# Xiaoming-Zhao/PointNav-VO

Hardware: AMD Instinct MI355X
Metric: RGB-D frame-pair VO inferences/s @341x192 (higher is better)
Workload: dtype f32

## Files before the change

pointnav-vo_amd/csrc/conv_x3.hip:

```cpp
#include <cmath>
#include <cstdio>
#include <cstdlib>
#include <cstring>

#include "pnvo_internal.h"

namespace pnvo {

typedef float f32x16 __attribute__((ext_vector_type(16)));
typedef float f32x4 __attribute__((ext_vector_type(4)));
typedef float f32x2 __attribute__((ext_vector_type(2)));
typedef __bf16 bf16x8 __attribute__((ext_vector_type(8)));
typedef __bf16 bf16x2 __attribute__((ext_vector_type(2)));
typedef _Float16 f16x8 __attribute__((ext_vector_type(8)));
typedef _Float16 f16x2 __attribute__((ext_vector_type(2)));
typedef unsigned u32x4 __attribute__((ext_vector_type(4)));

namespace {
__device__ __forceinline__ unsigned pack2(float a, float b) {
  const bf16x2 r = __builtin_convertvector(f32x2{a, b}, bf16x2);
  return __builtin_bit_cast(unsigned, r);
}
__device__ __forceinline__ unsigned pack2h(float a, float b) {
  const f16x2 r = __builtin_convertvector(f32x2{a, b}, f16x2);
  return __builtin_bit_cast(unsigned, r);
}
__device__ __forceinline__ float lo_f(unsigned u) { return __builtin_bit_cast(float, u << 16); }
__device__ __forceinline__ float hi_f(unsigned u) { return __builtin_bit_cast(float, u & 0xffff0000u); }
}

constexpr int x3_wpe(int mw, int nw, int np, bool dsf = false) {
  return dsf ? (mw * nw >= 6 ? 1 : (mw * nw >= 2 ? 2 : 3)) : ((np == 2 && mw * nw <= 2) ? 3 : 2);
}

template <int KS, int STRIDE, int MODE, int MW, int NW, int NP, bool DSF = false, bool W8 = false, bool KSW = false, bool M16 = false>
__global__ __launch_bounds__(W8 ? 512 : 256) __attribute__((amdgpu_waves_per_eu(W8 ? 2 : x3_wpe(MW, NW, NP, DSF), W8 ? 2 : x3_wpe(MW, NW, NP, DSF)))) void conv_x3_kernel(const ConvX3Args p) {
  constexpr int NTH = W8 ? 512 : 256, NWV = NTH / 64;
  constexpr int EMW = KSW ? 1 : MW;
  constexpr int NWT = M16 ? NW / 2 : NW;
  constexpr int TW = M16 ? (MW * NW + 3) / 4 : MW * NW;
  static_assert(!M16 || (NP == 2 && KS == 3 && STRIDE == 1 && !DSF && !KSW && NW % 2 == 0), "16x16x32 flavour: float16-piece 3x3 stride-1 convs, whole N-tiles");
  static_assert(!KSW || (NW == 1 && NP == 2 && KS == 3 && !DSF && !W8), "K split over the waves: float16-piece 3x3 convs, one N-tile");
  static_assert(!DSF || (KS == 3 && STRIDE == 2 && NP == 2 && (MODE == 0 || MODE == 2)), "the downsample rides on a float16-piece 3x3 stride-2 conv");
  extern __shared__ __attribute__((aligned(16))) unsigned char lds[];
  constexpr int PSTEP = KS == 1 ? STRIDE : 1;
  constexpr int CS = KS == 1 ? 1 : STRIDE;
  constexpr int PAD = KS / 2;
  const int lane = threadIdx.x & 63;
  const int wave = __builtin_amdgcn_readfirstlane(threadIdx.x >> 6);

  const int ntiles = p.B * p.tiles_r * p.tiles_c;
  const int chunk = (ntiles + 7) >> 3;
  int bid = (int)(blockIdx.x & 7) * chunk + (int)(blockIdx.x >> 3);
  if (bid >= ntiles) return;
  const int tci = bid % p.tiles_c;
  bid /= p.tiles_c;
  const int tri = bid % p.tiles_r;
  const int n = bid / p.tiles_r;
  const int r0 = tri * p.TR, c0 = tci * p.TC;
  const int hi0 = r0 * STRIDE - PAD, wi0 = c0 * STRIDE - PAD;
  const int mdl = (p.grp_end0 > 0 && n >= p.grp_end0) + (p.grp_end1 > 0 && n >= p.grp_end1);
  const unsigned short *g_wpk = mdl == 0 ? p.wpk : p.wpk_g[mdl - 1];
  const unsigned short *g_ds_wpk = mdl == 0 ? p.ds_wpk : p.ds_wpk_g[mdl - 1];
  const float g_oscale = mdl == 0 ? p.oscale : p.oscale_g[mdl - 1], g_ds_oscale = mdl == 0 ? p.ds_oscale : p.ds_oscale_g[mdl - 1];
  const float *g_gamma = mdl == 0 ? p.gn_gamma : p.gn_gamma_g[mdl - 1], *g_beta = mdl == 0 ? p.gn_beta : p.gn_beta_g[mdl - 1];
  const float *g_ds_gamma = mdl == 0 ? p.ds_gamma : p.ds_gamma_g[mdl - 1], *g_ds_beta = mdl == 0 ? p.ds_beta : p.ds_beta_g[mdl - 1];
  const int PR = p.PR, PC = p.PC, CK = p.CK;
  const int pitch = CK * 2 + 16;
  const int plane = PR * PC * pitch;
  const int npix = p.TR * p.TC;
  const int tab_off = KSW ? max(NP * plane, 4 * MW * 4096) : NP * plane;
  unsigned *qtab = reinterpret_cast<unsigned *>(lds + tab_off);
  unsigned *otab = qtab + p.MT * 32;
  for (int e = (int)threadIdx.x; e < p.MT * 32; e += NTH) {
    const int q = min(e, npix - 1);
    const int tr = q / p.TC, tc = q - tr * p.TC;
    qtab[e] = (unsigned)(((tr * CS) * PC + tc * CS) * pitch);
    const bool ok = e < npix && r0 + tr < p.Ho && c0 + tc < p.Wo;
    otab[e] = (unsigned)((tr * p.Wo + tc) * p.COUTP) | (ok ? 0u : 0x80000000u);
  }

  const int wn = p.wn;
  const int wave_m = wave / wn;
  const int wave_n = (wave & (wn - 1)) + (int)blockIdx.y * wn;
  const int ntt = p.COUTP >> 5, kct = p.CIN >> 4;

  f32x16 acc[MW][NW];
#pragma unroll
  for (int i = 0; i < MW; ++i)
#pragma unroll
    for (int j = 0; j < NW; ++j)
#pragma unroll
      for (int r = 0; r < 16; ++r) acc[i][j][r] = 0.f;
  f32x4 acc16[M16 ? MW : 1][M16 ? NW : 1];
  const int mt16 = (npix + 15) >> 4;
  const int m16_row = (mt16 + NWV / wn - 1) / (NWV / wn), m16_sub0 = wave_m * m16_row;
  const bool m16_last = m16_sub0 + MW <= mt16 && MW <= m16_row;
  if (M16) {
#pragma unroll
    for (int i = 0; i < MW; ++i)
#pragma unroll
      for (int j = 0; j < NW; ++j) acc16[M16 ? i : 0][M16 ? j : 0] = f32x4{0.f, 0.f, 0.f, 0.f};
  }
  f32x16 accd[DSF ? MW : 1][DSF ? NW : 1];
  if (DSF) {
#pragma unroll
    for (int i = 0; i < MW; ++i)
#pragma unroll
      for (int j = 0; j < NW; ++j)
#pragma unroll
        for (int r = 0; r < 16; ++r) accd[DSF ? i : 0][DSF ? j : 0][r] = 0.f;
  }

  float in_mul = 1.f, in_div = 1.f;
  const bool in_scaled = NP == 2 && p.in_absmax != nullptr;
  if (in_scaled) {
    unsigned mb = p.in_absmax[(threadIdx.x & 63) * 16];
#pragma unroll
    for (int d = 32; d >= 1; d >>= 1) mb = max(mb, (unsigned)__shfl_xor((int)mb, d));
    const int e = mb != 0u ? (int)((mb >> 23) & 0xffu) - 126 : 14;
    in_mul = __builtin_bit_cast(float, (unsigned)(14 - e + 127) << 23);
    in_div = __builtin_bit_cast(float, (unsigned)(e - 14 + 127) << 23);
  }
  const int G = CK >> 3;
  const int cg = threadIdx.x & (G - 1), pl = threadIdx.x / G, PS = NTH / G;
  const int dr = PS / PC, dc = PS - dr * PC;
  const int nppix = PR * PC;

  unsigned long long c_stage = 0, c_mm = 0, t_0 = __builtin_readcyclecounter(), r_0 = wall_clock64();
  for (int ck0 = 0; ck0 < p.CIN; ck0 += CK) {
    unsigned long long t_a = __builtin_readcyclecounter();
    if (ck0 > 0) __syncthreads();
    {
      f32x4 sc0, sc1, sh0, sh1, rs0, rs1, rt0, rt1;
      const bool res_ss = MODE == 2 && p.res_scale != nullptr;
      auto load_ss = [&]() {
        if (MODE >= 1) {
          const float *ps = p.in_scale + (long)n * p.CIN + ck0 + 8 * cg;
          const float *pt = p.in_shift + (long)n * p.CIN + ck0 + 8 * cg;
          sc0 = *reinterpret_cast<const f32x4 *>(ps);
          sc1 = *reinterpret_cast<const f32x4 *>(ps + 4);
          sh0 = *reinterpret_cast<const f32x4 *>(pt);
          sh1 = *reinterpret_cast<const f32x4 *>(pt + 4);
        }
        if (res_ss) {
          const float *ps = p.res_scale + (long)n * p.CIN + ck0 + 8 * cg;
          const float *pt = p.res_shift + (long)n * p.CIN + ck0 + 8 * cg;
          rs0 = *reinterpret_cast<const f32x4 *>(ps);
          rs1 = *reinterpret_cast<const f32x4 *>(ps + 4);
          rt0 = *reinterpret_cast<const f32x4 *>(pt);
          rt1 = *reinterpret_cast<const f32x4 *>(pt + 4);
        }
      };
      load_ss();
      int pr = pl / PC, pc = pl - pr * PC;
      const long img = ((long)n * p.H * p.W) * p.CIN + ck0 + 8 * cg;
      const float *xb = p.x + img;
      struct Round {
        f32x4 v[2][2], w[2][2];
        unsigned off[2];
        int gofs[2];
        bool ok[2], in[2], own[2];
      };
      auto fetch = [&](int pix, Round &r) {
#pragma unroll
        for (int k = 0; k < 2; ++k) {
          const int hi = hi0 + pr * PSTEP, wi = wi0 + pc * PSTEP;
          r.ok[k] = pix + k * PS < nppix;
          r.in[k] = r.ok[k] && hi >= 0 && hi < p.H && wi >= 0 && wi < p.W;
          r.off[k] = (unsigned)((pr * PC + pc) * pitch + 16 * cg);
          r.v[k][0] = r.v[k][1] = f32x4{0.f, 0.f, 0.f, 0.f};
          if (MODE >= 2) {
            r.own[k] = r.in[k] && p.xout != nullptr && blockIdx.y == 0 && pr >= PAD && pr < PAD + p.TR * CS && pc >= PAD && pc < PAD + p.TC * CS;
            r.gofs[k] = (hi * p.W + wi) * p.CIN;
          }
          if (r.in[k]) {
            const float *src = xb + ((long)hi * p.W + wi) * p.CIN;
            r.v[k][0] = *reinterpret_cast<const f32x4 *>(src);
            r.v[k][1] = *reinterpret_cast<const f32x4 *>(src + 4);
            if (MODE == 2) {
              const float *rsrc = p.res + img + ((long)hi * p.W + wi) * p.CIN;
              r.w[k][0] = *reinterpret_cast<const f32x4 *>(rsrc);
              r.w[k][1] = *reinterpret_cast<const f32x4 *>(rsrc + 4);
            }
          }
          pr += dr;
          pc += dc;
          if (pc >= PC) {
            pc -= PC;
            pr += 1;
          }
        }
      };
      auto split_store = [&](const Round &r) {
#pragma unroll
        for (int k = 0; k < 2; ++k) {
          if (!r.ok[k]) continue;
          float f[8];
#pragma unroll
          for (int e = 0; e < 8; ++e) {
            float t = r.v[k][e >> 2][e & 3];
            if (MODE == 1) {
              const f32x4 &sc = e < 4 ? sc0 : sc1, &sh = e < 4 ? sh0 : sh1;
              t = r.in[k] ? fmaxf(__builtin_fmaf(t, sc[e & 3], sh[e & 3]), 0.f) : 0.f;
            }
            if (MODE == 3) {
              const f32x4 &sc = e < 4 ? sc0 : sc1, &sh = e < 4 ? sh0 : sh1;
              int key = __builtin_bit_cast(int, t);
              key = key >= 0 ? key : key ^ 0x7fffffff;
              t = r.in[k] ? fmaxf(__builtin_fmaf(__builtin_bit_cast(float, key), __builtin_fabsf(sc[e & 3]), sh[e & 3]), 0.f) : 0.f;
            }
            if (MODE == 2) {
              const f32x4 &sc = e < 4 ? sc0 : sc1, &sh = e < 4 ? sh0 : sh1;
              float u = r.w[k][e >> 2][e & 3];
              if (res_ss) u = __builtin_fmaf(u, (e < 4 ? rs0 : rs1)[e & 3], (e < 4 ? rt0 : rt1)[e & 3]);
              t = r.in[k] ? fmaxf(__builtin_fmaf(t, sc[e & 3], sh[e & 3]) + u, 0.f) : 0.f;
            }
            f[e] = t;
          }
          if (MODE >= 2 && r.own[k]) {
            float *dst = p.xout + img + r.gofs[k];
            *reinterpret_cast<f32x4 *>(dst) = f32x4{f[0], f[1], f[2], f[3]};
            *reinterpret_cast<f32x4 *>(dst + 4) = f32x4{f[4], f[5], f[6], f[7]};
          }
          if (NP == 2) {
            if (in_scaled) {
#pragma unroll
              for (int e = 0; e < 8; ++e) f[e] *= in_mul;
            }
            u32x4 o0, o1;
#pragma unroll
            for (int e = 0; e < 4; ++e) {
              const float a = f[2 * e], b = f[2 * e + 1];
              const f16x2 h = __builtin_convertvector(f32x2{a, b}, f16x2);
              o0[e] = __builtin_bit_cast(unsigned, h);
              o1[e] = pack2h(a - (float)h[0], b - (float)h[1]);
            }
            *reinterpret_cast<u32x4 *>(lds + r.off[k]) = o0;
            *reinterpret_cast<u32x4 *>(lds + plane + r.off[k]) = o1;
            continue;
          }
          u32x4 o0, o1, o2;
#pragma unroll
          for (int e = 0; e < 4; ++e) {
            const float a = f[2 * e], b = f[2 * e + 1];
            const unsigned h = pack2(a, b);
            const float ra = a - lo_f(h), rb = b - hi_f(h);
            const unsigned m = pack2(ra, rb);
            o0[e] = h;
            o1[e] = m;
            o2[e] = pack2(ra - lo_f(m), rb - hi_f(m));
          }
          *reinterpret_cast<u32x4 *>(lds + r.off[k]) = o0;
          *reinterpret_cast<u32x4 *>(lds + plane + r.off[k]) = o1;
          *reinterpret_cast<u32x4 *>(lds + 2 * plane + r.off[k]) = o2;
        }
      };
      constexpr bool PIPE = !((MODE == 2 && (TW >= 6 || (M16 && !W8) || x3_wpe(MW, NW, NP) == 3 || DSF)) || (DSF && MW * NW == 4));
      if (TW <= 2 && !(MODE == 2 && (x3_wpe(MW, NW, NP) == 3 || DSF))) {
        for (int pix = pl; pix < nppix; pix += 6 * PS) {
          Round r0, r1, r2;
          fetch(pix, r0);
          fetch(pix + 2 * PS, r1);
          fetch(pix + 4 * PS, r2);
          split_store(r0);
          split_store(r1);
          split_store(r2);
        }
      } else if (PIPE) {
        Round cur, nxt;
        fetch(pl, cur);
        for (int pix = pl; pix < nppix; pix += 2 * PS) {
          const bool more = pix + 2 * PS < nppix;
          if (more) fetch(pix + 2 * PS, nxt);
          split_store(cur);
          if (more) cur = nxt;
        }
      } else {
        for (int pix = pl; pix < nppix; pix += 2 * PS) {
          Round cur;
          fetch(pix, cur);
          split_store(cur);
        }
      }
    }
    __syncthreads();
    unsigned long long t_b = __builtin_readcyclecounter();
    c_stage += t_b - t_a;

    if constexpr (M16) {
      unsigned aoff[MW];
#pragma unroll
      for (int i = 0; i < MW; ++i) {
        const int sub = min(m16_sub0 + i, mt16 - 1);
        aoff[i] = qtab[sub * 16 + (lane & 15)] + (unsigned)((lane >> 4) * 16);
      }
      const int kcc = CK >> 4, kcp = CK >> 5;
      const int nsteps = KS * KS * kcp;
      const unsigned kstep = (unsigned)ntt * (NP * 1024u);
      const char *wb_n = reinterpret_cast<const char *>(g_wpk) + (long)(ck0 >> 4) * kstep;
      unsigned toff_n = 0;
      int kc_n = 0, kw_n = 0;
      auto advance = [&]() {
        ++kc_n;
        toff_n += 64;
        wb_n += 2 * kstep;
        if (kc_n == kcp) {
          kc_n = 0;
          toff_n += (unsigned)(pitch - kcp * 64);
          wb_n += (long)(kct - kcc) * kstep;
          if (++kw_n == KS) {
            kw_n = 0;
            toff_n += (unsigned)((PC - KS) * pitch);
          }
        }
      };
      const int kg = lane >> 4;
      unsigned voff[NW];
#pragma unroll
      for (int j = 0; j < NW; ++j)
        voff[j] = (unsigned)min(wave_n * NWT + (j >> 1), ntt - 1) * (NP * 1024u) + (unsigned)(kg >> 1) * kstep +
                  (unsigned)((kg & 1) * 32 + 16 * (j & 1) + (lane & 15)) * 16u;
      auto loadA = [&](int i, u32x4 (*a)[MW]) {
#pragma unroll
        for (int pc = 0; pc < NP; ++pc) a[pc][i] = *reinterpret_cast<const u32x4 *>(lds + pc * plane + aoff[i] + toff_n);
      };
      auto loadB = [&](u32x4 (*b)[NW]) {
#pragma unroll
        for (int j = 0; j < NW; ++j)
#pragma unroll
          for (int pc = 0; pc < NP; ++pc) b[pc][j] = *reinterpret_cast<const u32x4 *>(wb_n + (size_t)voff[j] + pc * 1024);
      };
      auto step = [&](u32x4 (*a)[MW], const u32x4 (*b)[NW]) {
#pragma unroll
        for (int i = 0; i < MW; ++i) {
          if (i == MW - 1 && !m16_last) break;
          constexpr int TA[3] = {1, 0, 0}, TB[3] = {0, 1, 0};
#pragma unroll
          for (int jt = 0; jt < NWT; ++jt)
#pragma unroll
            for (int t = 0; t < 3; ++t)
#pragma unroll
              for (int j = 2 * jt; j < 2 * jt + 2; ++j)
                acc16[M16 ? i : 0][M16 ? j : 0] = __builtin_amdgcn_mfma_f32_16x16x32_f16(__builtin_bit_cast(f16x8, a[TA[t]][i]), __builtin_bit_cast(f16x8, b[TB[t]][M16 ? j : 0]),
                                                                                         acc16[M16 ? i : 0][M16 ? j : 0], 0, 0, 0);
          __builtin_amdgcn_sched_barrier(0);
          loadA(i, a);
          __builtin_amdgcn_sched_barrier(0);
        }
      };
      u32x4 a[NP][MW], b0[NP][NW], b1[NP][NW];
      loadB(b0);
#pragma unroll
      for (int i = 0; i < MW; ++i) loadA(i, a);
      advance();
#pragma unroll 1
      for (int s = 0; s < nsteps; s += 2) {
        loadB(b1);
        __builtin_amdgcn_sched_barrier(0);
        step(a, b0);
        if (s + 2 < nsteps) advance();
        if (s + 1 < nsteps) {
          loadB(b0);
          __builtin_amdgcn_sched_barrier(0);
          step(a, b1);
          if (s + 3 < nsteps) advance();
        }
      }
    } else {
    unsigned aoff[MW];
#pragma unroll
    for (int i = 0; i < MW; ++i) {
      const int mt = min(KSW ? i : wave_m * MW + i, p.MT - 1);
      aoff[i] = qtab[mt * 32 + (lane & 31)] + (unsigned)((lane >> 5) * 16);
    }
    const int kcc = CK >> 4;
    const int nsteps = KS * KS * kcc;
    const unsigned kstep = (unsigned)ntt * (NP * 1024u);
    const char *wb_n = reinterpret_cast<const char *>(g_wpk) + (long)(ck0 >> 4) * kstep;
    unsigned toff_n = 0;
    int kc_n = 0, kw_n = 0;
    auto advance = [&]() {
      ++kc_n;
      toff_n += 32;
      wb_n += kstep;
      if (kc_n == kcc) {
        kc_n = 0;
        toff_n += (unsigned)(pitch - kcc * 32);
        wb_n += (long)(kct - kcc) * kstep;
        if (++kw_n == KS) {
          kw_n = 0;
          toff_n += (unsigned)((PC - KS) * pitch);
        }
      }
    };
    constexpr bool RING = NP == 2 && KS == 3 && MW * NW <= 2;
    const char *wb_b = wb_n;
    int kc_b = 0;
    auto advanceB = [&]() {
      wb_b += kstep;
      if (++kc_b == kcc) {
        kc_b = 0;
        wb_b += (long)(kct - kcc) * kstep;
      }
    };
    unsigned voff[NW];
#pragma unroll
    for (int j = 0; j < NW; ++j) voff[j] = (unsigned)min(wave_n * NW + j, ntt - 1) * (NP * 1024u) + (unsigned)lane * 16u;
    auto loadBr = [&](u32x4 (*b)[NW]) {
#pragma unroll
      for (int j = 0; j < NW; ++j)
#pragma unroll
        for (int pc = 0; pc < NP; ++pc) b[pc][j] = *reinterpret_cast<const u32x4 *>(wb_b + (size_t)voff[j] + pc * 1024);
    };
    auto loadA = [&](int i, u32x4 (*a)[MW]) {
#pragma unroll
      for (int pc = 0; pc < NP; ++pc) a[pc][i] = *reinterpret_cast<const u32x4 *>(lds + pc * plane + aoff[i] + toff_n);
    };
    auto loadB = [&](u32x4 (*b)[NW]) {
#pragma unroll
      for (int j = 0; j < NW; ++j)
#pragma unroll
        for (int pc = 0; pc < NP; ++pc) b[pc][j] = *reinterpret_cast<const u32x4 *>(wb_n + (size_t)voff[j] + pc * 1024);
    };
    auto step = [&](u32x4 (*a)[MW], const u32x4 (*b)[NW]) {
#pragma unroll
      for (int i = 0; i < MW; ++i) {
#pragma unroll
        for (int j = 0; j < NW; ++j) {
          if (NP == 2) {
            constexpr int TA[3] = {1, 0, 0}, TB[3] = {0, 1, 0};
#pragma unroll
            for (int t = 0; t < 3; ++t)
              acc[i][j] = __builtin_amdgcn_mfma_f32_32x32x16_f16(__builtin_bit_cast(f16x8, a[TA[t]][i]),
                                                                 __builtin_bit_cast(f16x8, b[TB[t]][j]), acc[i][j], 0, 0, 0);
          } else {
            constexpr int TA[6] = {1, 2, 0, 1, 0, 0}, TB[6] = {1, 0, 2, 0, 1, 0};
#pragma unroll
            for (int t = 0; t < 6; ++t)
              acc[i][j] = __builtin_amdgcn_mfma_f32_32x32x16_bf16(__builtin_bit_cast(bf16x8, a[TA[t]][i]),
                                                                  __builtin_bit_cast(bf16x8, b[TB[t]][j]), acc[i][j], 0, 0, 0);
          }
        }
        __builtin_amdgcn_sched_barrier(0);
        loadA(i, a);
        __builtin_amdgcn_sched_barrier(0);
      }
    };
    u32x4 a[NP][MW], b0[NP][NW], b1[NP][NW];
    u32x4 bd0[DSF ? NP : 1][NW], bd1[DSF ? NP : 1][NW];
    auto loadBd = [&](u32x4 (*b)[NW], int kc) {
      const char *wd = reinterpret_cast<const char *>(g_ds_wpk) + (long)((ck0 >> 4) + kc) * kstep;
#pragma unroll
      for (int j = 0; j < NW; ++j)
#pragma unroll
        for (int pc = 0; pc < NP; ++pc) b[pc][j] = *reinterpret_cast<const u32x4 *>(wd + (size_t)voff[j] + pc * 1024);
    };
    if constexpr (KSW) {
      const int s0 = (wave * nsteps) >> 2, s1 = ((wave + 1) * nsteps) >> 2;
      {
        const int tap = s0 / kcc, kc = s0 - tap * kcc, kh = tap / KS, kw = tap - kh * KS;
        kc_n = kc;
        kw_n = kw;
        toff_n = (unsigned)((kh * PC + kw) * pitch + kc * 32);
        wb_n += ((long)tap * kct + kc) * kstep;
        kc_b = kc;
        wb_b = wb_n;
      }
      u32x4 br[3][NP][NW];
      int fb = s0;
      auto fetchB = [&](u32x4 (*bq)[NW]) {
        loadBr(bq);
        if (++fb < s1) advanceB();
      };
      fetchB(br[0]);
      fetchB(br[1]);
#pragma unroll
      for (int i = 0; i < MW; ++i) loadA(i, a);
      if (s0 + 1 < s1) advance();
#pragma unroll 1
      for (int s = s0; s < s1; s += 3) {
#pragma unroll
        for (int u = 0; u < 3; ++u) {
          if (s + u >= s1) break;
          fetchB(br[(u + 2) % 3]);
          __builtin_amdgcn_sched_barrier(0);
          step(a, br[u]);
          if (s + u + 2 < s1) advance();
        }
      }
    } else {
    if (DSF) loadBd(bd0, 0);
    loadB(b0);
#pragma unroll
    for (int i = 0; i < MW; ++i) loadA(i, a);
    advance();
    if (RING) {
      constexpr int R = MW * NW <= 2 ? 6 : 3;
      u32x4 br[R][NP][NW];
#pragma unroll
      for (int pc = 0; pc < NP; ++pc)
#pragma unroll
        for (int j = 0; j < NW; ++j) br[0][pc][j] = b0[pc][j];
#pragma unroll
      for (int q = 1; q < R - 1; ++q) {
        advanceB();
        loadBr(br[q]);
      }
      advanceB();
      constexpr bool A2 = MW * NW <= 2 && !(MODE == 2 && MW * NW == 2 && !DSF) && !(MODE == 2 && DSF && MW * NW == 1);
      u32x4 a1[A2 ? NP : 1][MW];
      if (A2) {
#pragma unroll
        for (int i = 0; i < MW; ++i) loadA(i, a1);
        advance();
      }
#pragma unroll 1
      for (int s = 0; s < nsteps; s += R) {
// ... 39 lines not shown
        constexpr int TA[3] = {1, 0, 0}, TB[3] = {0, 1, 0};
#pragma unroll
        for (int i = 0; i < MW; ++i)
#pragma unroll
          for (int j = 0; j < NW; ++j)
#pragma unroll
            for (int t = 0; t < 3; ++t)
              accd[i][j] = __builtin_amdgcn_mfma_f32_32x32x16_f16(__builtin_bit_cast(f16x8, ad[TA[t]][i]), __builtin_bit_cast(f16x8, bd[TB[t]][j]),
                                                                  accd[i][j], 0, 0, 0);
      };
      if constexpr (MW * NW == 4) {
#pragma unroll 1
        for (int kc = 0; kc < kcc; ++kc) {
          loadAd(kc);
          mm(bd0);
          if (kc + 1 < kcc) loadBd(bd0, kc + 1);
        }
      } else {
#pragma unroll 1
        for (int kc = 0; kc < kcc; kc += 2) {
          loadAd(kc);
          loadBd(bd1, kc + 1);
          mm(bd0);
          loadAd(kc + 1);
          if (kc + 2 < kcc) loadBd(bd0, kc + 2);
          mm(bd1);
        }
      }
    }
    }
    c_mm += __builtin_readcyclecounter() - t_b;
  }
  if constexpr (KSW) {
    __syncthreads();
    float *part = reinterpret_cast<float *>(lds);
#pragma unroll
    for (int i = 0; i < MW; ++i)
#pragma unroll
      for (int r = 0; r < 16; ++r) part[((wave * MW + i) * 16 + r) * 64 + lane] = acc[i][0][r];
    __syncthreads();
    const int mt = min(wave, MW - 1);
#pragma unroll
    for (int r = 0; r < 16; ++r) {
      float v = part[((0 * MW + mt) * 16 + r) * 64 + lane];
#pragma unroll
      for (int w = 1; w < 4; ++w) v += part[((w * MW + mt) * 16 + r) * 64 + lane];
      acc[0][0][r] = v;
    }
    __syncthreads();
  }
  unsigned long long t_e = __builtin_readcyclecounter();

  const int rr16 = lane >> 5;
  const long ybase = (((long)n * p.Ho + r0) * p.Wo + c0) * p.COUTP;
  auto put_stats = [&](const float *t1, const float *t2, float *stats, const float *gamma, const float *beta, float *gscale, float *gshift, float *gmu,
                       float *grstd) {
    if (stats != nullptr) {
      const int rows = NWV / wn;
      float *red = reinterpret_cast<float *>(lds);
      if (rows > 1) {
        __syncthreads();
        if (lane < 32)
#pragma unroll
          for (int j = 0; j < NWT; ++j) *reinterpret_cast<f32x2 *>(red + ((wave * NWT + j) * 32 + lane) * 2) = f32x2{t1[j], t2[j]};
        __syncthreads();
      }
      if (wave_m == 0 && lane < 32) {
#pragma unroll
        for (int j = 0; j < NWT; ++j) {
          const int nt = wave_n * NWT + j;
          if (nt >= ntt) continue;
          float s1 = t1[j], s2 = t2[j];
          for (int w = 1; w < rows; ++w) {
            const f32x2 o = *reinterpret_cast<const f32x2 *>(red + (((w * wn + (wave & (wn - 1))) * NWT + j) * 32 + lane) * 2);
            s1 += o[0];
            s2 += o[1];
          }
          float *dst = stats + (((long)n * p.slots + tri * p.tiles_c + tci) * p.COUTP + nt * 32 + lane) * 2;
          dst[0] = s1;
          dst[1] = s2;
          if (gscale != nullptr) {
            const int c = nt * 32 + lane;
            const bool first = gmu != nullptr && c % p.gn_cpg == 0;
            const long gi = (long)n * (p.COUTP / p.gn_cpg) + c / p.gn_cpg;
            gn_finalize_lane(s1, s2, p.gn_cpg, p.gn_P, p.gn_eps, gamma[c], beta[c], gscale + (long)n * p.COUTP + c,
                             gshift + (long)n * p.COUTP + c, first ? gmu + gi : nullptr, first ? grstd + gi : nullptr);
          }
        }
      }
    }
  };
  auto emit = [&](f32x16 (*ac)[NW], float *yout, float *stats, const float *oscale_ptr, float oscale, const float *gamma, const float *beta,
                  float *gscale, float *gshift, float *gmu, float *grstd, bool again) {
    if (NP == 2) {
      const float os = (oscale_ptr != nullptr ? *oscale_ptr : oscale) * in_div;
#pragma unroll
      for (int i = 0; i < EMW; ++i)
#pragma unroll
        for (int j = 0; j < NW; ++j)
#pragma unroll
          for (int r = 0; r < 16; ++r) ac[i][j][r] *= os;
    }
    float t1[NW], t2[NW];
#pragma unroll
    for (int j = 0; j < NW; ++j) t1[j] = t2[j] = 0.f;
#pragma unroll
    for (int i = 0; i < EMW; ++i) {
      const int mt = KSW ? wave : wave_m * MW + i;
      if (mt >= p.MT) continue;
      u32x4 ent[4];
#pragma unroll
      for (int g4 = 0; g4 < 4; ++g4) ent[g4] = *reinterpret_cast<const u32x4 *>(otab + mt * 32 + 8 * g4 + 4 * rr16);
      unsigned flags = 0;
#pragma unroll
      for (int g4 = 0; g4 < 4; ++g4) flags |= ent[g4][0] | ent[g4][1] | ent[g4][2] | ent[g4][3];
      const bool whole = !__any((int)(flags >> 31));
#pragma unroll
      for (int j = 0; j < NW; ++j) {
        const int nt = wave_n * NW + j;
        if (nt >= ntt) continue;
        const int co = nt * 32 + (lane & 31);
        float s1 = 0.f, s2 = 0.f;
        if (whole) {
#pragma unroll
          for (int r = 0; r < 16; ++r) {
            const float v = ac[i][j][r];
            (yout + ybase + co)[ent[r >> 2][r & 3]] = v;
            s1 += v;
            s2 = __builtin_fmaf(v, v, s2);
          }
        } else {
#pragma unroll
          for (int r = 0; r < 16; ++r) {
            const unsigned e = ent[r >> 2][r & 3];
            const bool ok = (int)e >= 0;
            const float v = ok ? ac[i][j][r] : 0.f;
            if (ok) (yout + ybase + co)[e] = v;
            s1 += v;
            s2 = __builtin_fmaf(v, v, s2);
          }
        }
        t1[j] += s1 + __shfl_xor(s1, 32);
        t2[j] += s2 + __shfl_xor(s2, 32);
      }
    }
    put_stats(t1, t2, stats, gamma, beta, gscale, gshift, gmu, grstd);
    (void)again;
  };
  if constexpr (M16) {
    const float os = (p.oscale_ptr != nullptr ? *p.oscale_ptr : g_oscale) * in_div;
    float t1[NWT], t2[NWT];
#pragma unroll
    for (int j = 0; j < NWT; ++j) t1[j] = t2[j] = 0.f;
    const bool upper = (lane & 16) != 0;
#pragma unroll
    for (int i = 0; i < MW; ++i) {
      const int sub = m16_sub0 + i;
      if (sub >= mt16 || (i == MW - 1 && !m16_last)) continue;
      const u32x4 ent = *reinterpret_cast<const u32x4 *>(otab + sub * 16 + 4 * (lane >> 4));
      const bool whole = !__any((int)((ent[0] | ent[1] | ent[2] | ent[3]) >> 31));
      auto sub_tile = [&](int j, float &s1, float &s2) {
#pragma clang fp contract(off)
        const int co = (wave_n * NWT + (j >> 1)) * 32 + 16 * (j & 1) + (lane & 15);
        s1 = s2 = 0.f;
#pragma unroll
        for (int r = 0; r < 4; ++r) {
          const unsigned e = ent[r];
          const bool ok = whole || (int)e >= 0;
          const float v = ok ? acc16[M16 ? i : 0][M16 ? j : 0][r] * os : 0.f;
          if (ok) (p.y + ybase + co)[e] = v;
          s1 += v;
          s2 = __builtin_fmaf(v, v, s2);
        }
        s1 += __shfl_xor(s1, 16);
        s2 += __shfl_xor(s2, 16);
        s1 += __shfl_xor(s1, 32);
        s2 += __shfl_xor(s2, 32);
      };
#pragma unroll
      for (int j = 0; j < NWT; ++j) {
        if (wave_n * NWT + j >= ntt) continue;
        float a1, a2, b1, b2;
        sub_tile(2 * j, a1, a2);
        sub_tile(2 * j + 1, b1, b2);
        t1[j] += upper ? b1 : a1;
        t2[j] += upper ? b2 : a2;
      }
    }
    put_stats(t1, t2, p.stats, g_gamma, g_beta, p.gn_scale, p.gn_shift, p.gn_mu, p.gn_rstd);
  } else
  emit(acc, p.y, p.stats, p.oscale_ptr, g_oscale, g_gamma, g_beta, p.gn_scale, p.gn_shift, p.gn_mu, p.gn_rstd, false);
  if constexpr (DSF) emit(accd, p.ds_y, p.ds_stats, p.ds_oscale_ptr, g_ds_oscale, g_ds_gamma, g_ds_beta, p.ds_scale, p.ds_shift, p.ds_mu, p.ds_rstd, true);
  if (p.prof && lane == 0 && blockIdx.x == 13 && blockIdx.y == 0) {
    const unsigned long long t_f = __builtin_readcyclecounter();
    unsigned long long *d = p.prof + wave * 8;
    d[0] = c_stage;
    d[1] = c_mm;
    d[2] = t_f - t_e;
    d[3] = t_f - t_0;
    d[4] = wall_clock64() - r_0;
  }
}


template <int MODE, int MW, int NW, bool BRES>
__global__ __launch_bounds__(256) __attribute__((amdgpu_waves_per_eu(BRES ? 2 : 3, BRES ? 2 : 3))) void conv_x3p_kernel(const ConvX3Args p) {
  static_assert(MODE == 0 || MODE == 1 || MODE == 3, "the block-tail stager has no registers for a second patch");
  static_assert(!BRES || NW == 1, "resident weights: one N-tile");
  extern __shared__ __attribute__((aligned(16))) unsigned char lds[];
  constexpr int KS = 3, PAD = 1, NP = 2;
  const int lane = threadIdx.x & 63;
  const int wave = __builtin_amdgcn_readfirstlane(threadIdx.x >> 6);
  const int ntiles = p.B * p.tiles_r * p.tiles_c;
  const int chunk = (ntiles + 7) >> 3;
  const int PR = p.PR, PC = p.PC, CK = p.CK;
  const int pitch = CK * 2 + 16;
  const int plane = PR * PC * pitch;
  const int npix = p.TR * p.TC;
  unsigned *qtab = reinterpret_cast<unsigned *>(lds + NP * plane);
  unsigned *otab = qtab + p.MT * 32;
  const int wn = p.wn;
  const int wave_m = wave / wn;
  const int wave_n = (wave & (wn - 1)) + (int)blockIdx.y * wn;
  const int ntt = p.COUTP >> 5;
  float in_mul = 1.f, in_div = 1.f;
  const bool in_scaled = p.in_absmax != nullptr;
  if (in_scaled) {
    unsigned mb = p.in_absmax[(threadIdx.x & 63) * 16];
#pragma unroll
    for (int d = 32; d >= 1; d >>= 1) mb = max(mb, (unsigned)__shfl_xor((int)mb, d));
    const int e = mb != 0u ? (int)((mb >> 23) & 0xffu) - 126 : 14;
    in_mul = __builtin_bit_cast(float, (unsigned)(14 - e + 127) << 23);
    in_div = __builtin_bit_cast(float, (unsigned)(e - 14 + 127) << 23);
  }
  const int G = CK >> 3;
  const int cg = threadIdx.x & (G - 1), pl = threadIdx.x / G, PS = 256 / G;
  const int nppix = PR * PC;
  constexpr int NPX = 6;
  int ppr[NPX], ppc[NPX];
  unsigned poff[NPX];
  bool pok[NPX];
#pragma unroll
  for (int k = 0; k < NPX; ++k) {
    const int pix = pl + k * PS;
    pok[k] = pix < nppix;
// ... 314 lines not shown
  int P, KS, STRIDE, NP, MODE, MW, NW, DSF, W8, KSW, M16;
  bool operator==(const X3Key &o) const { return std::memcmp(this, &o, sizeof(X3Key)) == 0; }
};
struct X3Instance {
  X3Key key;
  int threads;
  hipError_t (*launch)(const ConvX3Args &a, dim3 grid, size_t lds_bytes, hipStream_t s);
};
template <int P, int KS, int STRIDE, int NP, int MODE, int MW, int NW, bool DSF, bool W8, bool KSW, bool M16>
hipError_t x3_launch(const ConvX3Args &a, dim3 grid, size_t lds_bytes, hipStream_t s) {
  if constexpr (P != 0)
    hipLaunchKernelGGL((conv_x3p_kernel<MODE, MW, NW, true>), grid, dim3(256), lds_bytes, s, a);
  else
    hipLaunchKernelGGL((conv_x3_kernel<KS, STRIDE, MODE, MW, NW, NP, DSF, W8, KSW, M16>), grid, dim3(W8 ? 512 : 256), lds_bytes, s, a);
  return hipGetLastError();
}
#define X3I(P, KS, ST, NP, MODE, MW, NW, DSF, W8, KSW, M16) \
  {{P, KS, ST, NP, MODE, MW, NW, DSF, W8, KSW, M16}, (W8) ? 512 : 256, x3_launch<P, KS, ST, NP, MODE, MW, NW, DSF, W8, KSW, M16>},
#define X3_MODES(KS, ST, NP, MW, NW, DSF, W8, KSW, M16)    \
  X3I(0, KS, ST, NP, 0, MW, NW, DSF, W8, KSW, M16) X3I(0, KS, ST, NP, 1, MW, NW, DSF, W8, KSW, M16) \
  X3I(0, KS, ST, NP, 2, MW, NW, DSF, W8, KSW, M16) X3I(0, KS, ST, NP, 3, MW, NW, DSF, W8, KSW, M16)
#define X3_TILES(KS, ST, NP, MODE, DSF)                    \
  X3I(0, KS, ST, NP, MODE, 1, 1, DSF, 0, 0, 0) X3I(0, KS, ST, NP, MODE, 2, 1, DSF, 0, 0, 0) \
  X3I(0, KS, ST, NP, MODE, 2, 2, DSF, 0, 0, 0) X3I(0, KS, ST, NP, MODE, 3, 2, DSF, 0, 0, 0)
#define X3_GENERAL(KS, ST, NP) \
  X3_TILES(KS, ST, NP, 0, 0) X3_TILES(KS, ST, NP, 1, 0) X3_TILES(KS, ST, NP, 2, 0) X3_TILES(KS, ST, NP, 3, 0) X3_MODES(KS, ST, NP, 5, 1, 0, 0, 0, 0)
const X3Instance x3_table[] = {
  X3_GENERAL(3, 1, 2) X3_GENERAL(3, 2, 2) X3_GENERAL(1, 2, 2) X3_GENERAL(3, 1, 3) X3_GENERAL(3, 2, 3) X3_GENERAL(1, 2, 3)
  X3_TILES(3, 2, 2, 0, 1) X3_TILES(3, 2, 2, 2, 1)
  X3I(0, 3, 2, 2, 0, 3, 1, 1, 1, 0, 0) X3I(0, 3, 2, 2, 2, 3, 1, 1, 1, 0, 0)
  X3_MODES(3, 1, 2, 3, 1, 0, 1, 0, 0) X3_MODES(3, 2, 2, 3, 1, 0, 1, 0, 0)
  X3_MODES(3, 1, 2, 5, 2, 0, 1, 0, 1) X3_MODES(3, 1, 2, 5, 4, 0, 0, 0, 1) X3_MODES(3, 1, 2, 9, 2, 0, 0, 0, 1)
  X3I(0, 3, 1, 2, 0, 3, 1, 0, 0, 1, 0) X3I(0, 3, 1, 2, 1, 3, 1, 0, 0, 1, 0) X3I(0, 3, 1, 2, 2, 3, 1, 0, 0, 1, 0)
  X3I(0, 3, 1, 2, 0, 4, 1, 0, 0, 1, 0) X3I(0, 3, 1, 2, 1, 4, 1, 0, 0, 1, 0) X3I(0, 3, 1, 2, 2, 4, 1, 0, 0, 1, 0)
  X3I(1, 3, 1, 2, 0, 1, 1, 0, 0, 0, 0) X3I(1, 3, 1, 2, 1, 1, 1, 0, 0, 0, 0) X3I(1, 3, 1, 2, 0, 2, 1, 0, 0, 0, 0) X3I(1, 3, 1, 2, 1, 2, 1, 0, 0, 0, 0)
};
#undef X3_GENERAL
#undef X3_TILES
#undef X3_MODES
#undef X3I
constexpr int x3_table_rows = (int)(sizeof(x3_table) / sizeof(x3_table[0]));
int x3_find(const X3Key &k) {
  for (int i = 0; i < x3_table_rows; ++i)
    if (x3_table[i].key == k) return i;
  return -1;
}

ConvX3Plan tile_candidate(const ConvX3Problem &q, bool fine) {
  ConvX3Plan p;
  const int ks = q.ks, stride = q.stride;
  int mw = 0, nw = 0;
  if (q.CIN % 32 || q.COUTP % 32 || q.COUTP > 1024 || q.CIN > 1024) return {};
  if (!((ks == 3 && (stride == 1 || stride == 2)) || (ks == 1 && stride == 2))) return {};
  const int ntt = q.COUTP / 32;
  const bool strip_shape = q.opt.strip && !fine && q.np == 2 && stride == 1 && ks == 3 && ntt == 4 && q.Wo >= 16 && q.Ho >= 8;
  int TR, TC;
  if (stride == 2 && ks == 3) {
    TC = q.Wo >= 32 ? 16 : q.Wo;
    const int pc = 2 * TC + 1;
    TR = (324 / pc - 1) / 2;
    if (TR < 1) return {};
    if (TR > q.Ho) TR = q.Ho;
    while (TR > 1 && TR * TC > (ntt == 2 ? 64 : (ntt == 4 ? 128 : 96))) --TR;
  } else if (ntt == 1 && stride == 1 && ks == 3 && q.CIN > 32 && q.np == 2 && q.Wo < 32 && q.Ho * q.Wo <= 128) {
    TC = q.Wo;
    TR = q.Ho;
  } else if (ntt == 1) {
    if (stride != 1 || ks != 3 || q.CIN != 32) return {};
    TC = q.Wo >= 16 ? 16 : q.Wo;
    TR = 256 / TC;
    while (TR > 1 && (TR + 2) * (TC + 2) > 324) --TR;
    if (TR > q.Ho) TR = q.Ho;
    if (TR * TC <= 96) return {};
  } else if (strip_shape) {
    const int ncol = (q.Wo + 21) / 22;
    TC = (q.Wo + ncol - 1) / ncol;
    TR = 288 / TC;
    if (TR > q.Ho) TR = q.Ho;
    const int nrow = (q.Ho + TR - 1) / TR;
    TR = (q.Ho + nrow - 1) / nrow;
  } else if (q.Wo >= 32) {
    TR = 8;
    TC = 16;
  } else {
    TC = q.Wo;
    int target = ntt == 4 ? 192 : (ntt >= 8 ? 96 : 128);
    if (fine && q.opt.ksw && ks == 3 && stride == 1 && q.np == 2 && q.CIN >= 128) target = 96;
    TR = target / TC;
    if (TR < 1) TR = 1;
    if (TR > q.Ho) TR = q.Ho;
  }
  p.TR = TR;
  p.TC = TC;
  p.tiles_r = (q.Ho + TR - 1) / TR;
  p.tiles_c = (q.Wo + TC - 1) / TC;
  p.MT = (TR * TC + 31) / 32;
  const int cs = ks == 1 ? 1 : stride;
  p.PR = (TR - 1) * cs + ks;
  p.PC = (TC - 1) * cs + ks;
  const bool strip = strip_shape && p.MT > 6;
  if (fine) {
    if (p.MT > 8) return {};
    p.wn = 1;
    mw = (p.MT + 3) / 4;
    nw = 1;
    if (q.opt.ksw && (p.MT == 3 || p.MT == 4) && ks == 3 && stride == 1 && q.np == 2 && q.CIN >= 128) {
// ... 329 lines not shown
```

Measured before the change: 115,100.

## Use AMD buffer loads/stores with hardware bounds checks in conv_x3 kernel

Replaces global pointer loads and stores for input, residual, weights and outputs in the conv_x3 kernel with raw buffer resource loads and stores. Each resource is set up per image plane, and out-of-bounds offsets (a high-bit sentinel) return zero or drop the store in hardware. This removes the per-element branches, the zero-initialisation and the whole/partial tile split in staging and epilogue, and uses 32-bit offsets in place of 64-bit address arithmetic. Because offsets are now 32-bit, the planner gains a guard that rejects planes of 2GB or more; padded pixels are redirected to a trash LDS slot rather than skipped.

New measurement: 118,600, median of 6. 1.03x the previous value.

```diff
diff --git a/pointnav-vo_amd/csrc/conv_x3.hip b/pointnav-vo_amd/csrc/conv_x3.hip
--- a/pointnav-vo_amd/csrc/conv_x3.hip
+++ b/pointnav-vo_amd/csrc/conv_x3.hip
@@ -27,6 +27,19 @@
 }
 __device__ __forceinline__ float lo_f(unsigned u) { return __builtin_bit_cast(float, u << 16); }
 __device__ __forceinline__ float hi_f(unsigned u) { return __builtin_bit_cast(float, u & 0xffff0000u); }
+constexpr unsigned X3_OOB = 0x80000000u;
+__device__ __forceinline__ __amdgpu_buffer_rsrc_t x3_rsrc(const void *base, unsigned bytes) {
+  return __builtin_amdgcn_make_buffer_rsrc(const_cast<void *>(base), 0, bytes, 0x00020000);
+}
+__device__ __forceinline__ u32x4 x3_ldu(__amdgpu_buffer_rsrc_t r, unsigned voff, unsigned soff) {
+  return __builtin_bit_cast(u32x4, __builtin_amdgcn_raw_buffer_load_b128(r, voff, soff, 0));
+}
+__device__ __forceinline__ f32x4 x3_ldf(__amdgpu_buffer_rsrc_t r, unsigned voff) {
+  return __builtin_bit_cast(f32x4, __builtin_amdgcn_raw_buffer_load_b128(r, voff, 0, 0));
+}
+__device__ __forceinline__ void x3_stf(__amdgpu_buffer_rsrc_t r, unsigned voff, f32x4 v) {
+  __builtin_amdgcn_raw_buffer_store_b128(__builtin_bit_cast(u32x4, v), r, voff, 0, 0);
+}
 }
 
 constexpr int x3_wpe(int mw, int nw, int np, bool dsf = false) {
@@ -69,6 +82,17 @@
   const int pitch = CK * 2 + 16;
   const int plane = PR * PC * pitch;
   const int npix = p.TR * p.TC;
+  const unsigned xplane = (unsigned)(p.H * p.W * p.CIN) * 4u, yplane = (unsigned)(p.Ho * p.Wo * p.COUTP) * 4u;
+  const __amdgpu_buffer_rsrc_t rx = x3_rsrc(reinterpret_cast<const char *>(p.x) + (size_t)n * xplane, xplane);
+  const __amdgpu_buffer_rsrc_t rres = x3_rsrc(MODE == 2 ? reinterpret_cast<const char *>(p.res) + (size_t)n * xplane : nullptr, MODE == 2 ? xplane : 0u);
+  const bool xo = MODE >= 2 && p.xout != nullptr && blockIdx.y == 0;
+  const __amdgpu_buffer_rsrc_t rxo = x3_rsrc(xo ? reinterpret_cast<const char *>(p.xout) + (size_t)n * xplane : nullptr, xo ? xplane : 0u);
+  const __amdgpu_buffer_rsrc_t ry = x3_rsrc(reinterpret_cast<const char *>(p.y) + (size_t)n * yplane, yplane);
+  const __amdgpu_buffer_rsrc_t rdy = x3_rsrc(DSF ? reinterpret_cast<const char *>(p.ds_y) + (size_t)n * yplane : nullptr, DSF ? yplane : 0u);
+  const unsigned wbytes = (unsigned)(p.CIN >> 4) * (unsigned)(p.COUTP >> 5) * (NP * 1024u);
+  const __amdgpu_buffer_rsrc_t rw = x3_rsrc(g_wpk, (unsigned)(KS * KS) * wbytes);
+  const __amdgpu_buffer_rsrc_t rdw = x3_rsrc(DSF ? g_ds_wpk : nullptr, DSF ? wbytes : 0u);
+  const unsigned ytile = (unsigned)((r0 * p.Wo + c0) * p.COUTP) * 4u;
   const int tab_off = KSW ? max(NP * plane, 4 * MW * 4096) : NP * plane;
   unsigned *qtab = reinterpret_cast<unsigned *>(lds + tab_off);
   unsigned *otab = qtab + p.MT * 32;
@@ -77,7 +101,7 @@
     const int tr = q / p.TC, tc = q - tr * p.TC;
     qtab[e] = (unsigned)(((tr * CS) * PC + tc * CS) * pitch);
     const bool ok = e < npix && r0 + tr < p.Ho && c0 + tc < p.Wo;
-    otab[e] = (unsigned)((tr * p.Wo + tc) * p.COUTP) | (ok ? 0u : 0x80000000u);
+    otab[e] = ((unsigned)((tr * p.Wo + tc) * p.COUTP) * 4u) | (ok ? 0u : X3_OOB);
   }
 
   const int wn = p.wn;
@@ -126,6 +150,9 @@
   const int cg = threadIdx.x & (G - 1), pl = threadIdx.x / G, PS = NTH / G;
   const int dr = PS / PC, dc = PS - dr * PC;
   const int nppix = PR * PC;
+  const int pr_first = pl / PC, pc_first = pl - pr_first * PC;
+  const unsigned cin4 = (unsigned)p.CIN * 4u;
+  const unsigned trash = (unsigned)(min(pl, nppix - 1) * pitch + CK * 2);
 
   unsigned long long c_stage = 0, c_mm = 0, t_0 = __builtin_readcyclecounter(), r_0 = wall_clock64();
   for (int ck0 = 0; ck0 < p.CIN; ck0 += CK) {
@@ -153,36 +180,30 @@
         }
       };
       load_ss();
-      int pr = pl / PC, pc = pl - pr * PC;
-      const long img = ((long)n * p.H * p.W) * p.CIN + ck0 + 8 * cg;
-      const float *xb = p.x + img;
+      int pr = pr_first, pc = pc_first;
+      const unsigned cb = (unsigned)(ck0 + 8 * cg) * 4u;
       struct Round {
         f32x4 v[2][2], w[2][2];
-        unsigned off[2];
-        int gofs[2];
-        bool ok[2], in[2], own[2];
+        unsigned off[2], xofs[2];
+        bool in[2];
       };
       auto fetch = [&](int pix, Round &r) {
 #pragma unroll
         for (int k = 0; k < 2; ++k) {
           const int hi = hi0 + pr * PSTEP, wi = wi0 + pc * PSTEP;
-          r.ok[k] = pix + k * PS < nppix;
-          r.in[k] = r.ok[k] && hi >= 0 && hi < p.H && wi >= 0 && wi < p.W;
-          r.off[k] = (unsigned)((pr * PC + pc) * pitch + 16 * cg);
-          r.v[k][0] = r.v[k][1] = f32x4{0.f, 0.f, 0.f, 0.f};
+          const bool ok = pix + k * PS < nppix;
+          r.in[k] = ok && (unsigned)hi < (unsigned)p.H && (unsigned)wi < (unsigned)p.W;
+          r.off[k] = ok ? (unsigned)__umul24((unsigned)(pix + k * PS), (unsigned)pitch) + 16u * (unsigned)cg : trash;
+          const unsigned g = r.in[k] ? (unsigned)__umul24((unsigned)(__mul24(hi, p.W) + wi), cin4) + cb : X3_OOB;
           if (MODE >= 2) {
-            r.own[k] = r.in[k] && p.xout != nullptr && blockIdx.y == 0 && pr >= PAD && pr < PAD + p.TR * CS && pc >= PAD && pc < PAD + p.TC * CS;
-            r.gofs[k] = (hi * p.W + wi) * p.CIN;
+            const bool own = (unsigned)(pr - PAD) < (unsigned)(p.TR * CS) && (unsigned)(pc - PAD) < (unsigned)(p.TC * CS);
+            r.xofs[k] = own ? g : X3_OOB;
           }
-          if (r.in[k]) {
-            const float *src = xb + ((long)hi * p.W + wi) * p.CIN;
-            r.v[k][0] = *reinterpret_cast<const f32x4 *>(src);
-            r.v[k][1] = *reinterpret_cast<const f32x4 *>(src + 4);
-            if (MODE == 2) {
-              const float *rsrc = p.res + img + ((long)hi * p.W + wi) * p.CIN;
-              r.w[k][0] = *reinterpret_cast<const f32x4 *>(rsrc);
-              r.w[k][1] = *reinterpret_cast<const f32x4 *>(rsrc + 4);
-            }
+          r.v[k][0] = x3_ldf(rx, g);
+          r.v[k][1] = x3_ldf(rx, g + 16u);
+          if (MODE == 2) {
+            r.w[k][0] = x3_ldf(rres, g);
+            r.w[k][1] = x3_ldf(rres, g + 16u);
           }
           pr += dr;
           pc += dc;
@@ -195,7 +216,6 @@
       auto split_store = [&](const Round &r) {
 #pragma unroll
         for (int k = 0; k < 2; ++k) {
-          if (!r.ok[k]) continue;
           float f[8];
 #pragma unroll
           for (int e = 0; e < 8; ++e) {
@@ -218,12 +238,11 @@
             }
             f[e] = t;
           }
-          if (MODE >= 2 && r.own[k]) {
-            float *dst = p.xout + img + r.gofs[k];
-            *reinterpret_cast<f32x4 *>(dst) = f32x4{f[0], f[1], f[2], f[3]};
-            *reinterpret_cast<f32x4 *>(dst + 4) = f32x4{f[4], f[5], f[6], f[7]};
+          if (MODE >= 2) {
+            x3_stf(rxo, r.xofs[k], f32x4{f[0], f[1], f[2], f[3]});
+            x3_stf(rxo, r.xofs[k] + 16u, f32x4{f[4], f[5], f[6], f[7]});
           }
-          if (NP == 2) {
+          if constexpr (NP == 2) {
             if (in_scaled) {
 #pragma unroll
               for (int e = 0; e < 8; ++e) f[e] *= in_mul;
@@ -238,22 +257,22 @@
             }
             *reinterpret_cast<u32x4 *>(lds + r.off[k]) = o0;
             *reinterpret_cast<u32x4 *>(lds + plane + r.off[k]) = o1;
-            continue;
+          } else {
+            u32x4 o0, o1, o2;
+#pragma unroll
+            for (int e = 0; e < 4; ++e) {
+              const float a = f[2 * e], b = f[2 * e + 1];
+              const unsigned h = pack2(a, b);
+              const float ra = a - lo_f(h), rb = b - hi_f(h);
+              const unsigned m = pack2(ra, rb);
+              o0[e] = h;
+              o1[e] = m;
+              o2[e] = pack2(ra - lo_f(m), rb - hi_f(m));
+            }
+            *reinterpret_cast<u32x4 *>(lds + r.off[k]) = o0;
+            *reinterpret_cast<u32x4 *>(lds + plane + r.off[k]) = o1;
+            *reinterpret_cast<u32x4 *>(lds + 2 * plane + r.off[k]) = o2;
           }
-          u32x4 o0, o1, o2;
-#pragma unroll
-          for (int e = 0; e < 4; ++e) {
-            const float a = f[2 * e], b = f[2 * e + 1];
-            const unsigned h = pack2(a, b);
-            const float ra = a - lo_f(h), rb = b - hi_f(h);
-            const unsigned m = pack2(ra, rb);
-            o0[e] = h;
-            o1[e] = m;
-            o2[e] = pack2(ra - lo_f(m), rb - hi_f(m));
-          }
-          *reinterpret_cast<u32x4 *>(lds + r.off[k]) = o0;
-          *reinterpret_cast<u32x4 *>(lds + plane + r.off[k]) = o1;
-          *reinterpret_cast<u32x4 *>(lds + 2 * plane + r.off[k]) = o2;
         }
       };
       constexpr bool PIPE = !((MODE == 2 && (TW >= 6 || (M16 && !W8) || x3_wpe(MW, NW, NP) == 3 || DSF)) || (DSF && MW * NW == 4));
@@ -298,7 +317,7 @@
       const int kcc = CK >> 4, kcp = CK >> 5;
       const int nsteps = KS * KS * kcp;
       const unsigned kstep = (unsigned)ntt * (NP * 1024u);
-      const char *wb_n = reinterpret_cast<const char *>(g_wpk) + (long)(ck0 >> 4) * kstep;
+      unsigned wb_n = (unsigned)(ck0 >> 4) * kstep;
       unsigned toff_n = 0;
       int kc_n = 0, kw_n = 0;
       auto advance = [&]() {
@@ -308,7 +327,7 @@
         if (kc_n == kcp) {
           kc_n = 0;
           toff_n += (unsigned)(pitch - kcp * 64);
-          wb_n += (long)(kct - kcc) * kstep;
+          wb_n += (unsigned)(kct - kcc) * kstep;
           if (++kw_n == KS) {
             kw_n = 0;
             toff_n += (unsigned)((PC - KS) * pitch);
@@ -329,7 +348,7 @@
 #pragma unroll
         for (int j = 0; j < NW; ++j)
 #pragma unroll
-          for (int pc = 0; pc < NP; ++pc) b[pc][j] = *reinterpret_cast<const u32x4 *>(wb_n + (size_t)voff[j] + pc * 1024);
+          for (int pc = 0; pc < NP; ++pc) b[pc][j] = x3_ldu(rw, voff[j] + pc * 1024u, wb_n);
       };
       auto step = [&](u32x4 (*a)[MW], const u32x4 (*b)[NW]) {
 #pragma unroll
@@ -377,7 +396,7 @@
     const int kcc = CK >> 4;
     const int nsteps = KS * KS * kcc;
     const unsigned kstep = (unsigned)ntt * (NP * 1024u);
-    const char *wb_n = reinterpret_cast<const char *>(g_wpk) + (long)(ck0 >> 4) * kstep;
+    unsigned wb_n = (unsigned)(ck0 >> 4) * kstep;
     unsigned toff_n = 0;
     int kc_n = 0, kw_n = 0;
     auto advance = [&]() {
@@ -387,7 +406,7 @@
       if (kc_n == kcc) {
         kc_n = 0;
         toff_n += (unsigned)(pitch - kcc * 32);
-        wb_n += (long)(kct - kcc) * kstep;
+        wb_n += (unsigned)(kct - kcc) * kstep;
         if (++kw_n == KS) {
           kw_n = 0;
           toff_n += (unsigned)((PC - KS) * pitch);
@@ -395,13 +414,13 @@
       }
     };
     constexpr bool RING = NP == 2 && KS == 3 && MW * NW <= 2;
-    const char *wb_b = wb_n;
+    unsigned wb_b = wb_n;
     int kc_b = 0;
     auto advanceB = [&]() {
       wb_b += kstep;
       if (++kc_b == kcc) {
         kc_b = 0;
-        wb_b += (long)(kct - kcc) * kstep;
+        wb_b += (unsigned)(kct - kcc) * kstep;
       }
     };
     unsigned voff[NW];
@@ -411,7 +430,7 @@
 #pragma unroll
       for (int j = 0; j < NW; ++j)
 #pragma unroll
-        for (int pc = 0; pc < NP; ++pc) b[pc][j] = *reinterpret_cast<const u32x4 *>(wb_b + (size_t)voff[j] + pc * 1024);
+        for (int pc = 0; pc < NP; ++pc) b[pc][j] = x3_ldu(rw, voff[j] + pc * 1024u, wb_b);
     };
     auto loadA = [&](int i, u32x4 (*a)[MW]) {
 #pragma unroll
@@ -421,7 +440,7 @@
 #pragma unroll
       for (int j = 0; j < NW; ++j)
 #pragma unroll
-        for (int pc = 0; pc < NP; ++pc) b[pc][j] = *reinterpret_cast<const u32x4 *>(wb_n + (size_t)voff[j] + pc * 1024);
+        for (int pc = 0; pc < NP; ++pc) b[pc][j] = x3_ldu(rw, voff[j] + pc * 1024u, wb_n);
     };
     auto step = [&](u32x4 (*a)[MW], const u32x4 (*b)[NW]) {
 #pragma unroll
@@ -450,11 +469,11 @@
     u32x4 a[NP][MW], b0[NP][NW], b1[NP][NW];
     u32x4 bd0[DSF ? NP : 1][NW], bd1[DSF ? NP : 1][NW];
     auto loadBd = [&](u32x4 (*b)[NW], int kc) {
-      const char *wd = reinterpret_cast<const char *>(g_ds_wpk) + (long)((ck0 >> 4) + kc) * kstep;
+      const unsigned wd = (unsigned)((ck0 >> 4) + kc) * kstep;
 #pragma unroll
       for (int j = 0; j < NW; ++j)
 #pragma unroll
-        for (int pc = 0; pc < NP; ++pc) b[pc][j] = *reinterpret_cast<const u32x4 *>(wd + (size_t)voff[j] + pc * 1024);
+        for (int pc = 0; pc < NP; ++pc) b[pc][j] = x3_ldu(rdw, voff[j] + pc * 1024u, wd);
     };
     if constexpr (KSW) {
       const int s0 = (wave * nsteps) >> 2, s1 = ((wave + 1) * nsteps) >> 2;
@@ -463,7 +482,7 @@
         kc_n = kc;
         kw_n = kw;
         toff_n = (unsigned)((kh * PC + kw) * pitch + kc * 32);
-        wb_n += ((long)tap * kct + kc) * kstep;
+        wb_n += (unsigned)(tap * kct + kc) * kstep;
         kc_b = kc;
         wb_b = wb_n;
       }
@@ -609,7 +628,6 @@
   unsigned long long t_e = __builtin_readcyclecounter();
 
   const int rr16 = lane >> 5;
-  const long ybase = (((long)n * p.Ho + r0) * p.Wo + c0) * p.COUTP;
   auto put_stats = [&](const float *t1, const float *t2, float *stats, const float *gamma, const float *beta, float *gscale, float *gshift, float *gmu,
                        float *grstd) {
     if (stats != nullptr) {
@@ -647,7 +665,7 @@
       }
     }
   };
-  auto emit = [&](f32x16 (*ac)[NW], float *yout, float *stats, const float *oscale_ptr, float oscale, const float *gamma, const float *beta,
+  auto emit = [&](f32x16 (*ac)[NW], const __amdgpu_buffer_rsrc_t &ryo, float *stats, const float *oscale_ptr, float oscale, const float *gamma, const float *beta,
                   float *gscale, float *gshift, float *gmu, float *grstd, bool again) {
     if (NP == 2) {
       const float os = (oscale_ptr != nullptr ? *oscale_ptr : oscale) * in_div;
@@ -667,35 +685,20 @@
       if (mt >= p.MT) continue;
       u32x4 ent[4];
 #pragma unroll
-      for (int g4 = 0; g4 < 4; ++g4) ent[g4] = *reinterpret_cast<const u32x4 *>(otab + mt * 32 + 8 * g4 + 4 * rr16);
-      unsigned flags = 0;
-#pragma unroll
-      for (int g4 = 0; g4 < 4; ++g4) flags |= ent[g4][0] | ent[g4][1] | ent[g4][2] | ent[g4][3];
-      const bool whole = !__any((int)(flags >> 31));
+      for (int g4 = 0; g4 < 4; ++g4) ent[g4] = *reinterpret_cast<const u32x4 *>(otab + mt * 32 + 8 * g4 + 4 * rr16) + (unsigned)((lane & 31) * 4);
 #pragma unroll
       for (int j = 0; j < NW; ++j) {
         const int nt = wave_n * NW + j;
         if (nt >= ntt) continue;
-        const int co = nt * 32 + (lane & 31);
+        const unsigned so = ytile + (unsigned)nt * 128u;
         float s1 = 0.f, s2 = 0.f;
-        if (whole) {
-#pragma unroll
-          for (int r = 0; r < 16; ++r) {
-            const float v = ac[i][j][r];
-            (yout + ybase + co)[ent[r >> 2][r & 3]] = v;
-            s1 += v;
-            s2 = __builtin_fmaf(v, v, s2);
-          }
-        } else {
-#pragma unroll
-          for (int r = 0; r < 16; ++r) {
-            const unsigned e = ent[r >> 2][r & 3];
-            const bool ok = (int)e >= 0;
-            const float v = ok ? ac[i][j][r] : 0.f;
-            if (ok) (yout + ybase + co)[e] = v;
-            s1 += v;
-            s2 = __builtin_fmaf(v, v, s2);
-          }
+#pragma unroll
+        for (int r = 0; r < 16; ++r) {
+          const unsigned e = ent[r >> 2][r & 3];
+          const float v = (int)e >= 0 ? ac[i][j][r] : 0.f;
+          __builtin_amdgcn_raw_buffer_store_b32(__builtin_bit_cast(unsigned, v), ryo, e, so, 0);
+          s1 += v;
+          s2 = __builtin_fmaf(v, v, s2);
         }
         t1[j] += s1 + __shfl_xor(s1, 32);
         t2[j] += s2 + __shfl_xor(s2, 32);
@@ -714,18 +717,16 @@
     for (int i = 0; i < MW; ++i) {
       const int sub = m16_sub0 + i;
       if (sub >= mt16 || (i == MW - 1 && !m16_last)) continue;
-      const u32x4 ent = *reinterpret_cast<const u32x4 *>(otab + sub * 16 + 4 * (lane >> 4));
-      const bool whole = !__any((int)((ent[0] | ent[1] | ent[2] | ent[3]) >> 31));
+      const u32x4 ent = *reinterpret_cast<const u32x4 *>(otab + sub * 16 + 4 * (lane >> 4)) + (unsigned)((lane & 15) * 4);
       auto sub_tile = [&](int j, float &s1, float &s2) {
 #pragma clang fp contract(off)
-        const int co = (wave_n * NWT + (j >> 1)) * 32 + 16 * (j & 1) + (lane & 15);
+        const unsigned so = ytile + (unsigned)((wave_n * NWT + (j >> 1)) * 32 + 16 * (j & 1)) * 4u;
         s1 = s2 = 0.f;
 #pragma unroll
         for (int r = 0; r < 4; ++r) {
           const unsigned e = ent[r];
-          const bool ok = whole || (int)e >= 0;
-          const float v = ok ? acc16[M16 ? i : 0][M16 ? j : 0][r] * os : 0.f;
-          if (ok) (p.y + ybase + co)[e] = v;
+          const float v = (int)e >= 0 ? acc16[M16 ? i : 0][M16 ? j : 0][r] * os : 0.f;
+          __builtin_amdgcn_raw_buffer_store_b32(__builtin_bit_cast(unsigned, v), ry, e, so, 0);
           s1 += v;
           s2 = __builtin_fmaf(v, v, s2);
         }
@@ -746,8 +747,8 @@
     }
     put_stats(t1, t2, p.stats, g_gamma, g_beta, p.gn_scale, p.gn_shift, p.gn_mu, p.gn_rstd);
   } else
-  emit(acc, p.y, p.stats, p.oscale_ptr, g_oscale, g_gamma, g_beta, p.gn_scale, p.gn_shift, p.gn_mu, p.gn_rstd, false);
-  if constexpr (DSF) emit(accd, p.ds_y, p.ds_stats, p.ds_oscale_ptr, g_ds_oscale, g_ds_gamma, g_ds_beta, p.ds_scale, p.ds_shift, p.ds_mu, p.ds_rstd, true);
+  emit(acc, ry, p.stats, p.oscale_ptr, g_oscale, g_gamma, g_beta, p.gn_scale, p.gn_shift, p.gn_mu, p.gn_rstd, false);
+  if constexpr (DSF) emit(accd, rdy, p.ds_stats, p.ds_oscale_ptr, g_ds_oscale, g_ds_gamma, g_ds_beta, p.ds_scale, p.ds_shift, p.ds_mu, p.ds_rstd, true);
   if (p.prof && lane == 0 && blockIdx.x == 13 && blockIdx.y == 0) {
     const unsigned long long t_f = __builtin_readcyclecounter();
     unsigned long long *d = p.prof + wave * 8;
@@ -1168,6 +1169,7 @@
   int mw = 0, nw = 0;
   if (q.CIN % 32 || q.COUTP % 32 || q.COUTP > 1024 || q.CIN > 1024) return {};
   if (!((ks == 3 && (stride == 1 || stride == 2)) || (ks == 1 && stride == 2))) return {};
+  if ((long)q.H * q.W * q.CIN * 4 >= (1L << 31) || (long)q.Ho * q.Wo * q.COUTP * 4 >= (1L << 31)) return {};
   const int ntt = q.COUTP / 32;
   const bool strip_shape = q.opt.strip && !fine && q.np == 2 && stride == 1 && ks == 3 && ntt == 4 && q.Wo >= 16 && q.Ho >= 8;
   int TR, TC;
```
